# matchylabs/matchy

Hardware: AMD Instinct MI355X
Metric: log GB/s scanned (matchy match hot path, 100K IoCs) (higher is better)
Workload: dtype u8

## Files before the change

matchy_amd/csrc/device_common.h:

```cpp
#pragma once
#include <hip/hip_runtime.h>

#include "hashes.h"
#include "scan_types.h"

namespace mxy {

constexpr uint32_t C_B = 1, C_DIG = 2, C_DOT = 4, C_COLON = 8, C_AT = 16, C_LD = 32, C_NL = 64, C_TLD1 = 128;

constexpr uint64_t bnd_lo() {
    uint64_t m = 0;
    const int cs[] = {0x09, 0x0a, 0x0d, 0x20, 0x22, 0x27, 0x28, 0x29, 0x2c, 0x2f, 0x3a, 0x3b, 0x3c, 0x3d, 0x3e};
    for (int c : cs) m |= 1ull << c;
    return m;
}
constexpr uint64_t bnd_hi() {
    uint64_t m = 0;
    const int cs[] = {0x40, 0x5b, 0x5d, 0x7b, 0x7d};
    for (int c : cs) m |= 1ull << (c - 64);
    return m;
}
__device__ __forceinline__ bool d_is_boundary(uint32_t b) {
    if (b >= 128) return false;
    uint64_t m = b < 64 ? bnd_lo() : bnd_hi();
    return (m >> (b & 63)) & 1;
}
__device__ __forceinline__ bool d_is_digit(uint32_t b) { return b - '0' < 10u; }
__device__ __forceinline__ bool d_is_alpha(uint32_t b) { return (b | 0x20) - 'a' < 26u; }
__device__ __forceinline__ bool d_is_alnum(uint32_t b) { return d_is_digit(b) || d_is_alpha(b); }
__device__ __forceinline__ bool d_is_hex(uint32_t b) { return d_is_digit(b) || ((b | 0x20) - 'a' < 6u); }
__device__ __forceinline__ bool d_is_domain_char_fast(uint32_t b) { return d_is_alnum(b) || b == '-' || b == '.' || b >= 0x80; }
__device__ __forceinline__ bool d_is_domain_char(uint32_t b) { return d_is_alnum(b) || b == '-' || b == '.'; }
__device__ __forceinline__ bool d_is_email_local(uint32_t b) { return d_is_alnum(b) || b == '.' || b == '-' || b == '_' || b == '+'; }

__device__ __forceinline__ uint32_t class_of(uint32_t b) {
    uint32_t c = 0;
    if (d_is_boundary(b)) c |= C_B;
    if (d_is_digit(b)) c |= C_DIG;
    if (b == '.') c |= C_DOT;
    if (b == ':') c |= C_COLON;
    if (b == '@') c |= C_AT;
    if (d_is_alnum(b) || b >= 0x80) c |= C_LD;
    if (b == '\n') c |= C_NL;
    return c;
}

__device__ __forceinline__ uint32_t lane_id() { return __lane_id(); }
__device__ __forceinline__ uint64_t lanemask_lt() { return (1ull << lane_id()) - 1ull; }
__device__ __forceinline__ uint32_t mbcnt64_add(uint64_t m, uint32_t base) {
    return __builtin_amdgcn_mbcnt_hi((uint32_t)(m >> 32), __builtin_amdgcn_mbcnt_lo((uint32_t)m, base));
}
__device__ __forceinline__ uint32_t mbcnt64(uint64_t m) {
    return __builtin_amdgcn_mbcnt_hi((uint32_t)(m >> 32), __builtin_amdgcn_mbcnt_lo((uint32_t)m, 0u));
}

// ... 179 lines not shown
        const uint32_t n = (uint32_t)__popcll(m);
        if (left < n) {
            const uint32_t own = next == 0xFFFFFFFFu ? static_fn() : 0xFFFFFFFFu;
            pad_rest(out, cap);
            if (own != 0xFFFFFFFFu) {
                next = own;
                left = ANCHOR_CHUNK;
            } else {
                const uint32_t c = chunk_fn();
                uint32_t b = 0;
                uint32_t* const counter = counter_fn();
                if (lane_id() == 0) b = atomicAdd(counter, c);
                next = __builtin_amdgcn_readfirstlane(b);
                left = c;
            }
        }
        uint32_t slot = 0xFFFFFFFFu;
        if (emit) {
            slot = next + (uint32_t)__popcll(m & lanemask_lt());
            if (slot >= cap) slot = 0xFFFFFFFFu;
        }
        next += n;
        left -= n;
        return slot;
    }
};

struct LogView {
    const uint8_t* p;
    uint32_t len;
    __device__ __forceinline__ uint32_t at(uint32_t i) const { return p[i]; }
};

__device__ inline bool d_valid_utf8(const uint8_t* s, uint32_t n) {
    uint32_t i = 0;
    while (i < n) {
        uint32_t c = s[i];
        if (c < 0x80) { ++i; continue; }
        uint32_t l = (c >= 0xC2 && c <= 0xDF) ? 2 : (c >= 0xE0 && c <= 0xEF) ? 3 : (c >= 0xF0 && c <= 0xF4) ? 4 : 0;
        if (l == 0 || i + l > n) return false;
        uint32_t c1 = s[i + 1];
        uint32_t lo = 0x80, hi = 0xBF;
        if (c == 0xE0) lo = 0xA0;
        if (c == 0xED) hi = 0x9F;
        if (c == 0xF0) lo = 0x90;
        if (c == 0xF4) hi = 0x8F;
        if (c1 < lo || c1 > hi) return false;
        for (uint32_t k = 2; k < l; ++k) if ((s[i + k] & 0xC0) != 0x80) return false;
        i += l;
    }
    return true;
}

struct ByteMasks { uint64_t dc, dot, dash, high; };
struct ByteMasks32 { uint32_t dc, dot, dash, high; };
__device__ __forceinline__ ByteMasks32 domain_masks32(uint32_t x) {
    constexpr uint32_t H = 0x80808080u, L7 = 0x7F7F7F7Fu;
    const uint32_t t = x & L7, l = t | 0x20202020u;
    const uint32_t dig = (t + 0x50505050u) & ~(t + 0x46464646u);
    const uint32_t alp = (l + 0x1F1F1F1Fu) & ~(l + 0x05050505u);
    const uint32_t ndot = (t ^ 0x2E2E2E2Eu) + L7, ndash = (t ^ 0x2D2D2D2Du) + L7;
    ByteMasks32 m;
    m.high = x & H;
    m.dot = ~ndot & ~x & H;
    m.dash = ~ndash & ~x & H;
    m.dc = (((dig | alp) & ~x) | m.dot | m.dash | m.high) & H;
    return m;
}
__device__ __forceinline__ ByteMasks domain_masks(uint64_t x) {
    const ByteMasks32 lo = domain_masks32((uint32_t)x), hi = domain_masks32((uint32_t)(x >> 32));
    ByteMasks m;
    m.dc = (uint64_t)lo.dc | ((uint64_t)hi.dc << 32);
    m.dot = (uint64_t)lo.dot | ((uint64_t)hi.dot << 32);
    m.dash = (uint64_t)lo.dash | ((uint64_t)hi.dash << 32);
    m.high = (uint64_t)lo.high | ((uint64_t)hi.high << 32);
    return m;
}

__device__ __forceinline__ bool d_ipv4_from_window(uint4 q, uint32_t t4, uint32_t dot, uint32_t& start, uint32_t& end, uint32_t& addr) {
    const uint32_t b3 = q.x >> 24, b2 = (q.x >> 16) & 0xFF, b1 = (q.x >> 8) & 0xFF, b0 = q.x & 0xFF;
    if (!d_is_digit(b3)) return false;
    const bool g2 = d_is_digit(b2), g1 = g2 && d_is_digit(b1);
    const uint32_t n1 = 1u + g2 + g1;
    const uint32_t before = g1 ? b0 : g2 ? b1 : b2;
    if (!d_is_boundary(before)) return false;
    const uint32_t first = g1 ? b1 : g2 ? b2 : b3;
    uint32_t a = g1 ? (b1 - 48) * 100 + (b2 - 48) * 10 + (b3 - 48) : g2 ? (b2 - 48) * 10 + (b3 - 48) : (b3 - 48);
    if (a > 255 || (n1 > 1 && first == '0')) return false;
    uint32_t r0 = __builtin_amdgcn_alignbyte(q.z, q.y, 1), r1 = __builtin_amdgcn_alignbyte(q.w, q.z, 1), r2 = __builtin_amdgcn_alignbyte(t4, q.w, 1);
    uint32_t pos = dot + 1;
#pragma unroll
    for (int o = 0; o < 3; ++o) {
        const uint32_t c0 = r0 & 0xFF, c1 = (r0 >> 8) & 0xFF, c2 = (r0 >> 16) & 0xFF, c3 = r0 >> 24;
        if (!d_is_digit(c0)) return false;
        const bool h1 = d_is_digit(c1), h2 = h1 && d_is_digit(c2);
        const uint32_t n = 1u + h1 + h2;
        const uint32_t v = h2 ? (c0 - 48) * 100 + (c1 - 48) * 10 + (c2 - 48) : h1 ? (c0 - 48) * 10 + (c1 - 48) : (c0 - 48);
        if (v > 255 || (h1 && c0 == '0')) return false;
        const uint32_t sep = h2 ? c3 : h1 ? c2 : c1;
        a = (a << 8) | v;
        pos += n;
        if (o < 2) {
            if (sep != '.') return false;
            pos += 1;
            r0 = __builtin_amdgcn_alignbyte(r1, r0, n); r1 = __builtin_amdgcn_alignbyte(r2, r1, n); r2 = __builtin_amdgcn_alignbyte(0u, r2, n);
            r0 = __builtin_amdgcn_alignbyte(r1, r0, 1); r1 = __builtin_amdgcn_alignbyte(r2, r1, 1); r2 = r2 >> 8;
        } else if (!d_is_boundary(sep)) {
            return false;
        }
    }
    start = dot - n1; end = pos; addr = a;
    return true;
}
__device__ __forceinline__ bool val_ipv4_fast(const uint8_t* log, uint32_t dot, uint32_t& start, uint32_t& end, uint32_t& addr) {
    uint4 q;
    uint32_t t4;
    __builtin_memcpy(&q, log + dot - 4, 16);
    __builtin_memcpy(&t4, log + dot + 12, 4);
    return d_ipv4_from_window(q, t4, dot, start, end, addr);
}

__device__ inline bool val_ipv4(const LogView& lg, uint32_t dot, uint32_t& start, uint32_t& end, uint32_t& addr) {
    uint32_t s = dot;
    while (s > 0 && dot - s < 3 && d_is_digit(lg.at(s - 1))) --s;
    if (s == dot) return false;
    if (s > 0 && !d_is_boundary(lg.at(s - 1))) return false;
    uint32_t pos = s, a = 0;
    for (int idx = 0; idx < 4; ++idx) {
        uint32_t v = 0, digits = 0, first = 0;
        while (pos < lg.len && digits < 3) {
// ... 51 lines not shown
```

matchy_amd/csrc/hashes.h:

```cpp
#pragma once
#include <cstddef>
#include <cstdint>

#if defined(__HIPCC__)
#include <hip/hip_runtime.h>
#define MXY_HD __host__ __device__ inline __attribute__((always_inline))
#else
#define MXY_HD inline
#endif

namespace mxy {

MXY_HD uint64_t rotl64(uint64_t x, int r) { return (x << r) | (x >> (64 - r)); }

template <class Fetch>
MXY_HD uint64_t xxh64_fetch(Fetch f, size_t len, uint64_t seed) {
    const uint64_t P1 = 11400714785074694791ULL, P2 = 14029467366897019727ULL, P3 = 1609587929392839161ULL,
                   P4 = 9650029242287828579ULL, P5 = 2870177450012600261ULL;
    auto rd64 = [&](size_t o) {
        uint64_t v = 0;
        for (int k = 7; k >= 0; --k) v = (v << 8) | (uint64_t)f(o + k);
        return v;
    };
    auto rd32 = [&](size_t o) {
// ... 79 lines not shown
}

struct Xxh64Stream {
    static constexpr uint64_t P1 = 11400714785074694791ULL, P2 = 14029467366897019727ULL, P3 = 1609587929392839161ULL,
                              P4 = 9650029242287828579ULL, P5 = 2870177450012600261ULL;
    uint64_t v1, v2, v3, v4, lane[4] = {0, 0, 0, 0}, cur = 0, total = 0;
    uint32_t nlane = 0, ncur = 0;
    MXY_HD explicit Xxh64Stream(uint64_t seed) : v1(seed + P1 + P2), v2(seed + P2), v3(seed), v4(seed - P1) {}
    static MXY_HD uint64_t round(uint64_t acc, uint64_t in) { acc += in * P2; acc = rotl64(acc, 31); return acc * P1; }
    static MXY_HD uint64_t merge(uint64_t acc, uint64_t val) { val = round(0, val); acc ^= val; return acc * P1 + P4; }
    MXY_HD void push(uint32_t byte) {
        cur |= (uint64_t)(byte & 0xFF) << (8 * ncur);
        ++total;
        if (++ncur == 8) {
            lane[nlane] = cur; cur = 0; ncur = 0;
            if (++nlane == 4) {
                v1 = round(v1, lane[0]); v2 = round(v2, lane[1]); v3 = round(v3, lane[2]); v4 = round(v4, lane[3]);
                nlane = 0;
            }
        }
    }
    MXY_HD uint64_t finish(uint64_t seed) const {
        uint64_t h;
        if (total >= 32) {
            h = rotl64(v1, 1) + rotl64(v2, 7) + rotl64(v3, 12) + rotl64(v4, 18);
            h = merge(h, v1); h = merge(h, v2); h = merge(h, v3); h = merge(h, v4);
        } else {
            h = seed + P5;
        }
        h += total;
        for (uint32_t k = 0; k < nlane; ++k) { h ^= round(0, lane[k]); h = rotl64(h, 27) * P1 + P4; }
        uint64_t rest = cur;
        uint32_t n = ncur;
        if (n >= 4) { h ^= (rest & 0xFFFFFFFFull) * P1; h = rotl64(h, 23) * P2 + P3; rest >>= 32; n -= 4; }
        for (; n; --n) { h ^= (rest & 0xFF) * P5; h = rotl64(h, 11) * P1; rest >>= 8; }
        h ^= h >> 33; h *= P2; h ^= h >> 29; h *= P3; h ^= h >> 32;
        return h;
    }
};

MXY_HD uint32_t name_hash31(uint64_t l0, uint64_t l1, uint64_t l2, uint64_t l3, uint32_t n) {
    const uint64_t lane[4] = {l0, l1, l2, l3};
    uint32_t h = n * 0x9E3779B1u + 0x7F4A7C15u;
    for (int k = 0; k < 4; ++k) {
        const int rem = (int)n - 8 * k;
        const uint64_t m = rem >= 8 ? ~0ull : rem <= 0 ? 0ull : ((1ull << (8 * rem)) - 1ull);
        const uint64_t v = lane[k] & m;
        h = (h ^ (uint32_t)v) * 0x85EBCA6Bu; h ^= h >> 15;
        h = (h ^ (uint32_t)(v >> 32)) * 0xC2B2AE35u; h ^= h >> 13;
    }
    h *= 0x27D4EB2Fu; h ^= h >> 16;
    return h;
}

MXY_HD uint64_t fx_u32(uint32_t v) { return rotl64((uint64_t)v * 0xf1357aea2e62a9c5ULL, 26); }

constexpr uint32_t TLD_TAB_BITS = 11;
MXY_HD uint32_t tld_tab_slot(uint32_t lo, uint32_t hi24) { return ((lo ^ (hi24 * 0x9E3779B1u)) * 0x85EBCA6Bu) >> (32 - TLD_TAB_BITS); }

MXY_HD uint32_t tld_hash8(uint32_t lo, uint32_t hi) {
    uint32_t h = (lo * 0x9E3779B1u) ^ (hi * 0x85EBCA6Bu);
    h ^= h >> 16; h *= 0x7FEB352Du; h ^= h >> 15;
    return h;
}

MXY_HD uint64_t psl_hash_init() { return 0xcbf29ce484222325ULL; }
MXY_HD uint64_t psl_hash_step(uint64_t h, uint8_t b) { return (h ^ b) * 0x100000001b3ULL; }
MXY_HD uint64_t psl_hash_finish(uint64_t h) { h ^= h >> 29; h *= 0xbf58476d1ce4e5b9ULL; h ^= h >> 32; return h; }

}
```

matchy_amd/csrc/validate_kernels.hip:

```cpp
#include <hip/hip_runtime.h>

#include <cstdlib>

#include "hashes.h"
#include "scan_types.h"

#include "device_shared.h"

namespace mxy {


struct BackReader {
    const uint8_t* p;
    uint32_t pos;
    uint32_t cb;
    uint32_t k;
    uint64_t cur, nxt;
    __device__ __forceinline__ static uint64_t load8(const uint8_t* a) { uint64_t v; __builtin_memcpy(&v, a, 8); return v; }
    __device__ __forceinline__ void init(const uint8_t* base, uint32_t q) {
        p = base; pos = q; cb = 0; k = 0; cur = 0; nxt = 0;
        if (q >= 16) { cb = q - 8; k = 8; cur = load8(p + cb); nxt = load8(p + cb - 8); }
    }
    __device__ __forceinline__ uint32_t next() {
        --pos;
// ... 165 lines not shown
    }
    while (open && p < lg.len) {
        uint32_t c = lg.at(p);
        if (!d_is_domain_char_fast(c)) { stop_c = c; break; }
        if (c == '.') return false;
        if (p - j >= db.max_tld_len) return false;
        th = tld_hash_step(th, c);
        ++p;
    }
    const uint32_t e = p, ll = e - j;
    if (edge && stop_c == 0x100) *edge = true;
    if (ll > db.max_tld_len) return false;
    if (stop_c != 0x100 && !d_is_boundary(stop_c)) return false;
    bool alone = false;
    if (wide && ll <= 7) {
        const uint32_t lo = ll >= 4 ? w.x : (w.x & ((1u << (8 * ll)) - 1u));
        const uint32_t hi = ll > 4 ? (w.y & ((1u << (8 * (ll - 4))) - 1u)) : 0u;
        uint32_t slot = tld_tab_slot(lo, hi);
        for (;;) {
            const uint2 t = tldtab[slot];
            if ((t.y >> 24) == 0) return false;
            if (t.x == lo && (t.y & 0xFFFFFFu) == hi) { alone = (t.y >> 24) & 1; break; }
            slot = (slot + 1) & ((1u << TLD_TAB_BITS) - 1);
        }
    } else {
        const uint32_t bit = tld_hash_bit(th);
        if (!((bloom[bit >> 5] >> (bit & 31)) & 1)) return false;
    }
    uint32_t s;
    BackReader br;
    br.init(lg.p, e);
    WalkInit wi;
    wi.rh = psl_hash_init();
    WalkState ws{};
    const int r = alone ? domain_walk_back<false>(lg, db, min_labels, e, br, wi, s, long_out ? &ws : nullptr, nullptr, edge)
                        : domain_walk_back<true>(lg, db, min_labels, e, br, wi, s, long_out ? &ws : nullptr, nullptr, edge);
    if (r == WALK_LONG) { long_out->st = ws; long_out->e = e; long_out->alone = alone; return WALK_LONG; }
    if (r != WALK_YES) return WALK_NO;
    start = s; end = e;
    return WALK_YES;
}
__device__ bool val_domain_resume(const LogView& lg, const DevDb& db, uint32_t min_labels, const DomLong& dl, uint32_t& start, uint32_t& end, bool& need_utf8) {
    BackReader br;
    br.init(lg.p, dl.st.pos);
    WalkInit wi;
    wi.rh = psl_hash_init();
    wi.cur = dl.st.cur; wi.last_c = dl.st.last_c; wi.labels = dl.st.labels; wi.high = dl.st.high; wi.bad = dl.st.bad; wi.found = dl.st.found;
    uint32_t s;
    if (domain_walk_back<false>(lg, db, min_labels, dl.e, br, wi, s, nullptr, &need_utf8) != WALK_YES) return false;
    start = s; end = dl.e;
    return true;
}

__device__ __forceinline__ int val_domain_pre(const uint2* tldtab, uint32_t min_labels, uint32_t j, uint2 w, uint64_t b0, uint64_t b1,
                                              uint64_t b2, uint32_t& start, uint32_t& end) {
    constexpr uint64_t H = 0x8080808080808080ull;
    const uint64_t w64 = (uint64_t)w.x | ((uint64_t)w.y << 32);
    const ByteMasks mw = domain_masks(w64);
    const uint64_t ndc = ~mw.dc & H;
    const uint32_t ll = ndc ? (uint32_t)(__ffsll((long long)ndc) - 1) >> 3 : 8u;
    if (ll <= 7 && ll >= 1) {
        const uint64_t below = (1ull << (8 * ll)) - 1ull;
        if (mw.dot & below) return 0;
        const uint32_t stop_c = (uint32_t)(w64 >> (8 * ll)) & 0xFF;
        if (!d_is_boundary(stop_c)) return 0;
        const uint32_t lo = (uint32_t)(w64 & below), hi = (uint32_t)((w64 & below) >> 32);
        uint32_t slot = tld_tab_slot(lo, hi);
        bool alone = false;
        for (;;) {
            const uint2 t = tldtab[slot];
            if ((t.y >> 24) == 0) return 0;
            if (t.x == lo && (t.y & 0xFFFFFFu) == hi) { alone = (t.y >> 24) & 1; break; }
            slot = (slot + 1) & ((1u << TLD_TAB_BITS) - 1);
        }
        if (alone) {
            const ByteMasks m0 = domain_masks(b0), m1 = domain_masks(b1), m2 = domain_masks(b2);
            const uint64_t n0m = ~m0.dc & H, n1m = ~m1.dc & H, n2m = ~m2.dc & H;
            const uint32_t c0 = n0m ? (uint32_t)__clzll((long long)n0m) >> 3 : 8u;
            const uint32_t c1 = n1m ? (uint32_t)__clzll((long long)n1m) >> 3 : 8u, c2 = n2m ? (uint32_t)__clzll((long long)n2m) >> 3 : 8u;
            const uint32_t consumed = c0 < 8 ? c0 : (c1 < 8 ? 8 + c1 : 16 + c2);
            if (consumed < 24 || j == 24) {
                auto top = [](uint32_t k) -> uint64_t { return k == 0 ? 0ull : (~0ull << (64 - 8 * k)); };
                const uint64_t r0 = top(min(consumed, 8u)), r1 = top(consumed > 8 ? min(consumed - 8, 8u) : 0u),
                               r2 = top(consumed > 16 ? consumed - 16 : 0u);
                const uint64_t d0 = m0.dot >> 8, d1 = (m1.dot >> 8) | (m0.dot << 56), d2 = (m2.dot >> 8) | (m1.dot << 56);
                const uint64_t s0 = m0.dash >> 8, s1 = (m1.dash >> 8) | (m0.dash << 56), s2 = (m2.dash >> 8) | (m1.dash << 56);
                const uint64_t bad = ((m0.dot & (d0 | s0)) | (m0.dash & d0)) & r0;
                const uint64_t bad1 = ((m1.dot & (d1 | s1)) | (m1.dash & d1)) & r1, bad2 = ((m2.dot & (d2 | s2)) | (m2.dash & d2)) & r2;
                const uint32_t ndots = (uint32_t)(__popcll(m0.dot & r0) + __popcll(m1.dot & r1) + __popcll(m2.dot & r2));
                const uint32_t li = 24 - consumed;
                const uint64_t lw = li < 8 ? b2 : li < 16 ? b1 : b0;
                const uint32_t left_c = (uint32_t)(lw >> (8 * (li & 7))) & 0xFF;
                const uint32_t fi = 23 - consumed;
                const uint64_t fw = fi < 8 ? b2 : fi < 16 ? b1 : b0;
                const uint32_t first_c = consumed < 24 ? (uint32_t)(fw >> (8 * (fi & 7))) & 0xFF : 0x100u;
                const uint32_t lastc = (uint32_t)(w64 >> (8 * (ll - 1))) & 0xFF;
                const bool any_bad = (bad | bad1 | bad2) != 0 || lastc == '-' || consumed == 0 || left_c == '.' || left_c == '-';
                if (any_bad || ndots == 0 || 1 + ndots < min_labels) return 0;
                if (first_c != 0x100 && !d_is_boundary(first_c)) return 0;
                const uint32_t s_pos = j - consumed;
                const bool high = ((m0.high & r0) | (m1.high & r1) | (m2.high & r2) | (mw.high & below)) != 0;
                if (high) return 2;
                start = s_pos; end = j + ll;
                return 1;
            }
        }
    }
    return 2;
}

template <int NB>
__device__ __forceinline__ int val_domain_ctx(const uint2* tldtab, uint32_t min_labels, uint32_t j, uint2 w, const uint64_t (&b)[NB],
                                              uint32_t& start, uint32_t& end) {
    static_assert(NB >= 1 && NB <= 7, "a label must not reach 64 bytes inside the context");
    constexpr uint64_t H = 0x8080808080808080ull;
    const uint64_t w64 = (uint64_t)w.x | ((uint64_t)w.y << 32);
    const ByteMasks mw = domain_masks(w64);
    const uint64_t ndc = ~mw.dc & H;
    const uint32_t ll = ndc ? (uint32_t)(__ffsll((long long)ndc) - 1) >> 3 : 8u;
    if (ll > 7 || ll < 1) return 2;
    const uint64_t below = (1ull << (8 * ll)) - 1ull;
    if (mw.dot & below) return 0;
    const uint32_t stop_c = (uint32_t)(w64 >> (8 * ll)) & 0xFF;
    if (!d_is_boundary(stop_c)) return 0;
    const uint32_t lo = (uint32_t)(w64 & below), hi = (uint32_t)((w64 & below) >> 32);
    uint32_t slot = tld_tab_slot(lo, hi);
    bool alone = false;
    for (;;) {
        const uint2 t = tldtab[slot];
        if ((t.y >> 24) == 0) return 0;
        if (t.x == lo && (t.y & 0xFFFFFFu) == hi) { alone = (t.y >> 24) & 1; break; }
        slot = (slot + 1) & ((1u << TLD_TAB_BITS) - 1);
    }
    if (!alone) return 2;
    ByteMasks m[NB];
    uint32_t consumed = 0;
    bool open = true;
#pragma unroll
    for (int k = 0; k < NB; ++k) {
        m[k] = domain_masks(b[k]);
        const uint64_t nm = ~m[k].dc & H;
        const uint32_t ck = nm ? (uint32_t)__clzll((long long)nm) >> 3 : 8u;
        if (open) { consumed += ck; open = ck == 8; }
    }
    if (consumed == 8 * NB && j != 8 * NB) return 2;
    uint64_t bad = 0, high = mw.high & below;
    uint32_t ndots = 0;
#pragma unroll
    for (int k = 0; k < NB; ++k) {
        const uint32_t in_k = consumed > 8u * k ? min(consumed - 8u * k, 8u) : 0u;
        const uint64_t r = in_k == 0 ? 0ull : (~0ull << (64 - 8 * in_k));
        const uint64_t d = (m[k].dot >> 8) | (k ? (m[k ? k - 1 : 0].dot << 56) : 0ull);
        const uint64_t sd = (m[k].dash >> 8) | (k ? (m[k ? k - 1 : 0].dash << 56) : 0ull);
        bad |= ((m[k].dot & (d | sd)) | (m[k].dash & d)) & r;
        ndots += (uint32_t)__popcll(m[k].dot & r);
        high |= m[k].high & r;
    }
    const uint32_t li = 8 * NB - consumed, fi = li - 1;
    uint32_t left_c = 0, first_c = 0x100u;
#pragma unroll
    for (int k = 0; k < NB; ++k) {
        const uint32_t wi = (uint32_t)(NB - 1 - k);
// ... 421 lines not shown
    d_keccak256_1blk(dec, dl - 4, h);
    const uint32_t chk = (uint32_t)dec[dl - 4] | ((uint32_t)dec[dl - 3] << 8) | ((uint32_t)dec[dl - 2] << 16) | ((uint32_t)dec[dl - 1] << 24);
    return (uint32_t)h[0] == chk;
}
__device__ int d_bech32_val(uint32_t c) {
    const char* CS = "qpzry9x8gf2tvdw0s3jn54khce6mua7l";
    for (int i = 0; i < 32; ++i) if ((uint32_t)CS[i] == c) return i;
    return -1;
}
__device__ bool val_btc_bech32(const uint8_t* s, uint32_t n) {
    if (n < 3 + 6) return false;
    auto step = [](uint32_t chk, uint32_t v) {
        const uint32_t GEN[5] = {0x3b6a57b2, 0x26508e6d, 0x1ea119fa, 0x3d4233dd, 0x2a1462b3};
        uint32_t top = chk >> 25;
        chk = ((chk & 0x1ffffff) << 5) ^ v;
        for (int i = 0; i < 5; ++i) if ((top >> i) & 1) chk ^= GEN[i];
        return chk;
    };
    uint32_t chk = 1;
    chk = step(chk, 'b' >> 5); chk = step(chk, 'c' >> 5); chk = step(chk, 0); chk = step(chk, 'b' & 31); chk = step(chk, 'c' & 31);
    for (uint32_t k = 3; k < n; ++k) {
        int v = d_bech32_val(s[k]);
        if (v < 0) return false;
        chk = step(chk, (uint32_t)v);
    }
    return chk == 1 || chk == 0x2bc830a3u;
}
__device__ bool val_eth(const uint8_t* a, uint8_t* lower) {
    bool all_lower = true, all_upper = true;
    for (int i = 0; i < 40; ++i) {
        uint32_t c = a[2 + i];
        if (!d_is_hex(c)) return false;
        if (d_is_alpha(c)) { if (c >= 'a') all_upper = false; else all_lower = false; }
        lower[i] = (uint8_t)d_lower(c);
    }
    if (all_lower || all_upper) return true;
    uint64_t h[4];
    d_keccak256_1blk(lower, 40, h);
    for (int i = 0; i < 40; ++i) {
        uint32_t c = a[2 + i];
        if (d_is_alpha(c)) {
            const uint32_t byte = (uint32_t)(h[i >> 4] >> (8 * ((i >> 1) & 7))) & 0xFF;
            const uint32_t nib = (i & 1) ? (byte & 0x0f) : (byte >> 4);
            if ((c < 'a') != (nib >= 8)) return false;
        }
    }
    return true;
}

template <int MODE>
__global__ __launch_bounds__(256) void k_validate_dom(TokParams p, DevDb db) {
    constexpr bool AC = MODE == 1, SFX = MODE == 2;
    __shared__ uint2 tldtab[1u << TLD_TAB_BITS];
    __shared__ __attribute__((aligned(16))) uint32_t strbuf[256][8];
    __shared__ uint8_t dcls[AC ? 256 : 4];
    __shared__ uint32_t drows[AC ? DFA_LDS_ENTRIES_VAL : 1];
    for (uint32_t i = threadIdx.x; i < (1u << TLD_TAB_BITS); i += blockDim.x) tldtab[i] = db.tld_tab[i];
    DfaView dv{dcls, drows, 0};
    if constexpr (AC) dv = dfa_stage<DFA_LDS_ENTRIES_VAL>(db, dcls, drows);
    __syncthreads();
    ChunkWriter<Candidate, CAND_CHUNK> cw_dense;
    __shared__ Candidate wb_cand[4][64];
    BufferedWriter<Candidate> cw(wb_cand[threadIdx.x >> 6]);
    __shared__ RareAnchor wb_slow[4][64];
    BufferedWriter<RareAnchor> sw(wb_slow[threadIdx.x >> 6]);
    const Candidate SC{0, 0xFFFFFFFFu, 0, 0};
    const uint32_t stride = gridDim.x * blockDim.x;
    const uint32_t nd = min(p.counters->n_dom, p.dom_cap);
    struct Rec { uint32_t j; uint32_t c[8]; };
    auto load_rec = [&](uint32_t i, Rec& r) {
        r.j = 0xFFFFFFFFu;
#pragma unroll
        for (int k = 0; k < 8; ++k) r.c[k] = 0;
        if (i < nd) {
            r.j = p.dom_list[dom_plane_index(i, 0)];
#pragma unroll
            for (int k = 0; k < 8; ++k) r.c[k] = p.dom_list[dom_plane_index(i, 1 + k)];
        }
    };
    Rec cur, nxt;
    load_rec(blockIdx.x * blockDim.x + threadIdx.x, cur);
    {
        uint32_t g = cur.j;
#pragma unroll
        for (int k = 0; k < 8; ++k) g ^= cur.c[k];
        asm volatile("" ::"v"(g));
    }
    uint32_t pend_start = 0, pend_lt = 0, pend_word = 0xFFFFFFFFu, pend_bit = 0, n_valid = 0;
    uint32_t pend_sw[SFX ? 4 : 1] = {0}, pend_sb[SFX ? 4 : 1] = {0};
    bool pend = false, pend_over = false;
    uint32_t* sb = strbuf[threadIdx.x];
    auto queue_glob = [&](uint32_t b, uint32_t n) {
        if (!p.glob_work_d) return;
        const uint32_t lane = lane_id();
        const bool g = lane < n && b + lane < p.cand_cap && cw.buf[lane].pad == CAND_GLOB;
        const uint64_t m = __ballot(g);
        if (!m) return;
        uint32_t wb = 0;
        if (lane == 0) wb = atomicAdd(&p.counters->n_glob_work_d, (uint32_t)__popcll(m));
        wb = __builtin_amdgcn_readfirstlane(wb);
        const uint32_t slot = wb + mbcnt64(m);
        if (g && slot < p.glob_work_d_cap) p.glob_work_d[slot] = b + lane;
    };
    auto emit_pending = [&]() {
        if (!p.filter_lit) { cw_dense.append(pend, Candidate{pend_start, pend_lt, 0u, 0u}, p.cands, p.cand_cap, p.n_cand, SC); return; }
        bool lit = (pend_word >> pend_bit) & 1;
        uint32_t flag = 0;
        if constexpr (SFX) {
            bool g = pend_over;
#pragma unroll
            for (int q = 0; q < 4; ++q) g = g || ((pend_sw[q] >> pend_sb[q]) & 1);
            flag = g ? CAND_GLOB : CAND_NO_GLOB;
            lit = lit || g;
        }
        if constexpr (AC) flag = pend_over ? CAND_GLOB : CAND_NO_GLOB;
        if constexpr (AC || SFX) cw.append_then(pend && lit, Candidate{pend_start, pend_lt, 0u, flag}, p.cands, p.cand_cap, p.n_cand, queue_glob);
        else cw.append(pend && lit, Candidate{pend_start, pend_lt, 0u, flag}, p.cands, p.cand_cap, p.n_cand);
    };
    for (uint32_t base = blockIdx.x * blockDim.x; base < nd; base += stride) {
        const uint32_t i = base + threadIdx.x;
        emit_pending();
        pend = false;
        load_rec(i + stride, nxt);
        bool slow = false;
        if (cur.j != 0xFFFFFFFFu) {
            uint32_t s = 0, e = 0;
            int r = 2;
            if (!(cur.j & 0x80000000u)) {
                const uint64_t b2 = (uint64_t)cur.c[0] | ((uint64_t)cur.c[1] << 32), b1 = (uint64_t)cur.c[2] | ((uint64_t)cur.c[3] << 32),
                               b0 = (uint64_t)cur.c[4] | ((uint64_t)cur.c[5] << 32);
                r = val_domain_pre(tldtab, p.min_labels, cur.j, make_uint2(cur.c[6], cur.c[7]), b0, b1, b2, s, e);
            }
            slow = r == 2;
            if (r == 1) {
                pend_start = s; pend_lt = (e - s) | ((uint32_t)IT_DOMAIN << 24); pend = true;
                pend_word = 0xFFFFFFFFu; pend_bit = 0;
                n_valid += 1;
                if (p.filter_lit) {
                    *reinterpret_cast<uint4*>(sb) = make_uint4(cur.c[0], cur.c[1], cur.c[2], cur.c[3]);
                    *reinterpret_cast<uint4*>(sb + 4) = make_uint4(cur.c[4], cur.c[5], cur.c[6], cur.c[7]);
                    const uint32_t o = 24 - (cur.j - s), n = e - s;
                    const uint32_t i0 = o >> 2, sh = o & 3;
                    uint32_t wd[9];
#pragma unroll
                    for (int k = 0; k < 9; ++k) wd[k] = (i0 + k) < 8 ? sb[(i0 + k) & 7] : 0u;
                    uint64_t ln[4];
#pragma unroll
                    for (int k = 0; k < 4; ++k)
                        ln[k] = (uint64_t)__builtin_amdgcn_alignbyte(wd[2 * k + 1], wd[2 * k], sh) |
                                ((uint64_t)__builtin_amdgcn_alignbyte(wd[2 * k + 2], wd[2 * k + 1], sh) << 32);
                    if (db.ci) {
#pragma unroll
                        for (int k = 0; k < 4; ++k) ln[k] = ascii_lower8(ln[k]);
                    }
                    const uint32_t b = name_hash31(ln[0], ln[1], ln[2], ln[3], n) & db.lit_bm_mask;
                    pend_word = db.lit_bm ? db.lit_bm[b >> 5] : 0u;
                    pend_bit = b & 31;
                    if constexpr (SFX) {
                        const uint64_t fb = 0x0101010101010101ull * db.sfx_first;
                        uint32_t M = 0;
#pragma unroll
                        for (int k = 0; k < 4; ++k) {
                            const uint64_t x = ln[k] ^ fb;
                            const uint64_t z = ~(((x & 0x7F7F7F7F7F7F7F7Full) + 0x7F7F7F7F7F7F7F7Full) | x) & 0x8080808080808080ull;
                            const uint32_t lo = (uint32_t)z >> 7, hi = (uint32_t)(z >> 32) >> 7;
                            M |= ((((lo * 0x01020408u) >> 24) & 0xFu) | ((((hi * 0x01020408u) >> 24) & 0xFu) << 4)) << (8 * k);
                        }
                        M &= n >= 32 ? 0xFFFFFFFFu : ((1u << n) - 1u);
                        pend_over = false;
                        uint32_t dm = db.sfx_dots;
#pragma unroll
                        for (int q = 0; q < 4; ++q) {
                            pend_sw[q] = 0; pend_sb[q] = 0;
                            if (dm) {
                                const uint32_t d = (uint32_t)__builtin_ctz(dm) + 1;
                                dm &= dm - 1;
                                uint32_t m = M;
                                for (uint32_t j = 1; j < d; ++j) m &= ~(m ? (0x80000000u >> __builtin_clz(m)) : 0u);
                                if (m) {
                                    const uint32_t kk = 31u - (uint32_t)__builtin_clz(m), sl = n - kk;
                                    if (sl >= 3) {
                                        const uint32_t o2 = o + kk, j0 = o2 >> 2, s2 = o2 & 3;
                                        uint32_t w2[9];
#pragma unroll
                                        for (int k = 0; k < 9; ++k) w2[k] = (j0 + k) < 8 ? sb[(j0 + k) & 7] : 0u;
                                        uint64_t l2[4];
#pragma unroll
                                        for (int k = 0; k < 4; ++k)
                                            l2[k] = (uint64_t)__builtin_amdgcn_alignbyte(w2[2 * k + 1], w2[2 * k], s2) |
                                                    ((uint64_t)__builtin_amdgcn_alignbyte(w2[2 * k + 2], w2[2 * k + 1], s2) << 32);
                                        if (db.ci) {
#pragma unroll
                                            for (int k = 0; k < 4; ++k) l2[k] = ascii_lower8(l2[k]);
                                        }
                                        const uint32_t b2 = name_hash31(l2[0], l2[1], l2[2], l2[3], sl) & db.sfx_mask;
                                        pend_sw[q] = db.sfx_bm[b2 >> 5];
                                        pend_sb[q] = b2 & 31;
                                    }
                                }
                            }
                        }
                    }
                    if constexpr (AC) {
                        uint32_t st = 0, any = 0;
#pragma unroll
                        for (int k = 0; k < 31; ++k) {
                            const uint32_t c = dcls[(uint32_t)(ln[k >> 3] >> (8 * (k & 7))) & 0xFF];
                            if ((uint32_t)k < n) {
                                const uint32_t t = st < dv.lds_states ? drows[st * db.dfa_k + c] : db.dfa[(size_t)st * db.dfa_k + c];
                                st = t & 0x7FFFFFFFu;
                                any |= t;
                            }
                        }
                        pend_over = (any >> 31) != 0;
                        if (pend_over) { pend_word = 0xFFFFFFFFu; pend_bit = 0; }
                    }
                }
            }
        }
        sw.append(slow, RareAnchor{cur.j & 0x7FFFFFFFu, (uint32_t)RARE_DOM}, p.rare_dom, p.rare_dom_cap, &p.counters->n_rare_dom);
        cur = nxt;
    }
    emit_pending();
    if constexpr (AC || SFX) cw.flush_then(p.cands, p.cand_cap, p.n_cand, queue_glob);
    else cw.flush(p.cands, p.cand_cap, p.n_cand);
    cw_dense.pad_rest(p.cands, p.cand_cap, SC);
    sw.flush(p.rare_dom, p.rare_dom_cap, &p.counters->n_rare_dom);
#pragma unroll
    for (int off = 32; off > 0; off >>= 1) n_valid += __shfl_down(n_valid, off);
    if (lane_id() == 0 && n_valid) atomicAdd(&p.counters->cand_true, n_valid);
}

__device__ __forceinline__ bool lit_bm_may_hit(const DevDb& db, const LogView& lg, uint32_t s, uint32_t n, bool ascii) {
    uint64_t l[4] = {0, 0, 0, 0};
    if (s + 32 <= lg.len) {
#pragma unroll
        for (int k = 0; k < 4; ++k) __builtin_memcpy(&l[k], lg.p + s + 8 * k, 8);
    } else {
        for (uint32_t k = 0; k < 32 && s + k < lg.len; ++k) l[k >> 3] |= (uint64_t)lg.p[s + k] << (8 * (k & 7));
    }
    if (db.ci) {
        if (!ascii) {
            if (n > 32) return true;
            uint64_t high = 0;
#pragma unroll
            for (int k = 0; k < 4; ++k) {
                const int rem = (int)n - 8 * k;
                const uint64_t m = rem >= 8 ? ~0ull : (rem <= 0 ? 0ull : ((1ull << (8 * rem)) - 1ull));
// ... 373 lines not shown
```

Measured before the change: 2236.

## Rewrite domain pre-validation with bit-plane masks and register-only label alignment

```diff
diff --git a/matchy_amd/csrc/device_common.h b/matchy_amd/csrc/device_common.h
--- a/matchy_amd/csrc/device_common.h
+++ b/matchy_amd/csrc/device_common.h
@@ -1,6 +1,7 @@
 #pragma once
 #include <hip/hip_runtime.h>
 
+#include "domain_pre.h"
 #include "hashes.h"
 #include "scan_types.h"
 
@@ -286,30 +287,6 @@
     return true;
 }
 
-struct ByteMasks { uint64_t dc, dot, dash, high; };
-struct ByteMasks32 { uint32_t dc, dot, dash, high; };
-__device__ __forceinline__ ByteMasks32 domain_masks32(uint32_t x) {
-    constexpr uint32_t H = 0x80808080u, L7 = 0x7F7F7F7Fu;
-    const uint32_t t = x & L7, l = t | 0x20202020u;
-    const uint32_t dig = (t + 0x50505050u) & ~(t + 0x46464646u);
-    const uint32_t alp = (l + 0x1F1F1F1Fu) & ~(l + 0x05050505u);
-    const uint32_t ndot = (t ^ 0x2E2E2E2Eu) + L7, ndash = (t ^ 0x2D2D2D2Du) + L7;
-    ByteMasks32 m;
-    m.high = x & H;
-    m.dot = ~ndot & ~x & H;
-    m.dash = ~ndash & ~x & H;
-    m.dc = (((dig | alp) & ~x) | m.dot | m.dash | m.high) & H;
-    return m;
-}
-__device__ __forceinline__ ByteMasks domain_masks(uint64_t x) {
-    const ByteMasks32 lo = domain_masks32((uint32_t)x), hi = domain_masks32((uint32_t)(x >> 32));
-    ByteMasks m;
-    m.dc = (uint64_t)lo.dc | ((uint64_t)hi.dc << 32);
-    m.dot = (uint64_t)lo.dot | ((uint64_t)hi.dot << 32);
-    m.dash = (uint64_t)lo.dash | ((uint64_t)hi.dash << 32);
-    m.high = (uint64_t)lo.high | ((uint64_t)hi.high << 32);
-    return m;
-}
 
 __device__ __forceinline__ bool d_ipv4_from_window(uint4 q, uint32_t t4, uint32_t dot, uint32_t& start, uint32_t& end, uint32_t& addr) {
     const uint32_t b3 = q.x >> 24, b2 = (q.x >> 16) & 0xFF, b1 = (q.x >> 8) & 0xFF, b0 = q.x & 0xFF;
diff --git a/matchy_amd/csrc/domain_pre.h b/matchy_amd/csrc/domain_pre.h
--- /dev/null
+++ b/matchy_amd/csrc/domain_pre.h
@@ -0,0 +1,139 @@
+#pragma once
+#include <cstdint>
+
+#include "anchor_planes.h"
+#include "hashes.h"
+
+namespace mxy {
+
+struct ByteMasks { uint64_t dc, dot, dash, high; };
+struct ByteMasks32 { uint32_t dc, dot, dash, high; };
+MXY_HD ByteMasks32 domain_masks32(uint32_t x) {
+    constexpr uint32_t H = 0x80808080u, L7 = 0x7F7F7F7Fu;
+    const uint32_t t = x & L7, l = t | 0x20202020u;
+    const uint32_t dig = (t + 0x50505050u) & ~(t + 0x46464646u);
+    const uint32_t alp = (l + 0x1F1F1F1Fu) & ~(l + 0x05050505u);
+    const uint32_t ndot = (t ^ 0x2E2E2E2Eu) + L7, ndash = (t ^ 0x2D2D2D2Du) + L7;
+    ByteMasks32 m;
+    m.high = x & H;
+    m.dot = ~ndot & ~x & H;
+    m.dash = ~ndash & ~x & H;
+    m.dc = (((dig | alp) & ~x) | m.dot | m.dash | m.high) & H;
+    return m;
+}
+MXY_HD ByteMasks domain_masks(uint64_t x) {
+    const ByteMasks32 lo = domain_masks32((uint32_t)x), hi = domain_masks32((uint32_t)(x >> 32));
+    ByteMasks m;
+    m.dc = (uint64_t)lo.dc | ((uint64_t)hi.dc << 32);
+    m.dot = (uint64_t)lo.dot | ((uint64_t)hi.dot << 32);
+    m.dash = (uint64_t)lo.dash | ((uint64_t)hi.dash << 32);
+    m.high = (uint64_t)lo.high | ((uint64_t)hi.high << 32);
+    return m;
+}
+
+MXY_HD uint32_t byte_perm(uint32_t hi, uint32_t lo, uint32_t sel) {
+#if defined(__HIP_DEVICE_COMPILE__)
+    return __builtin_amdgcn_perm(hi, lo, sel);
+#else
+    const uint64_t v = ((uint64_t)hi << 32) | lo;
+    uint32_t r = 0;
+    for (int i = 0; i < 4; ++i) r |= (uint32_t)((v >> (8 * ((sel >> (8 * i)) & 7))) & 0xFF) << (8 * i);
+    return r;
+#endif
+}
+MXY_HD uint32_t byte_align(uint32_t hi, uint32_t lo, uint32_t sh) {
+#if defined(__HIP_DEVICE_COMPILE__)
+    return __builtin_amdgcn_alignbyte(hi, lo, sh);
+#else
+    return (uint32_t)((((uint64_t)hi << 32) | lo) >> (8 * (sh & 3)));
+#endif
+}
+
+struct CtxMasks {
+    uint32_t dc;
+    uint32_t dot;
+    uint32_t dash;
+    uint32_t high;
+    uint32_t bnd;
+};
+MXY_HD CtxMasks domain_ctx_masks(const uint32_t (&c)[8]) {
+    uint32_t r[8];
+#pragma unroll
+    for (int h = 0; h < 2; ++h) {
+        const uint32_t x0 = byte_perm(c[2 + h], c[h], 0x05010400u), x1 = byte_perm(c[2 + h], c[h], 0x07030602u);
+        const uint32_t y0 = byte_perm(c[6 + h], c[4 + h], 0x05010400u), y1 = byte_perm(c[6 + h], c[4 + h], 0x07030602u);
+        r[4 * h + 0] = byte_perm(y0, x0, 0x05040100u);
+        r[4 * h + 1] = byte_perm(y0, x0, 0x07060302u);
+        r[4 * h + 2] = byte_perm(y1, x1, 0x05040100u);
+        r[4 * h + 3] = byte_perm(y1, x1, 0x07060302u);
+    }
+    bit_transpose8(r);
+    const ClassPlanes cp = classify_planes(r, false);
+    CtxMasks m;
+    m.high = r[7];
+    m.dot = cp.T;
+    m.dash = andn(r[7] | r[6] | r[4] | r[1], r[5] & r[3] & r[2] & r[0]);
+    m.dc = cp.LD | cp.T | m.dash;
+    m.bnd = cp.B;
+    return m;
+}
+
+MXY_HD uint32_t ctx_label_len(const CtxMasks& m) { return (uint32_t)__builtin_ctz(~(m.dc >> 24)); }
+MXY_HD uint32_t ctx_label_lo(uint32_t w0, uint32_t ll) { return ll >= 4 ? w0 : (w0 & ((1u << (8 * ll)) - 1u)); }
+MXY_HD uint32_t ctx_label_hi(uint32_t w1, uint32_t ll) { return ll > 4 ? (w1 & ((1u << (8 * (ll - 4))) - 1u)) : 0u; }
+
+template <class TldEntry>
+MXY_HD int val_domain_pre(const TldEntry* tldtab, uint32_t min_labels, uint32_t j, const uint32_t (&c)[8], const CtxMasks& m,
+                          uint32_t& start, uint32_t& end) {
+    constexpr uint32_t FRONT = 0x00FFFFFFu;
+    const uint32_t ll = ctx_label_len(m);
+    if (ll > 7 || ll < 1) return 2;
+    const uint32_t lab = ((1u << ll) - 1u) << 24;
+    if (m.dot & lab) return 0;
+    if (!((m.bnd >> (24 + ll)) & 1u)) return 0;
+    const uint32_t lo = ctx_label_lo(c[6], ll), hi = ctx_label_hi(c[7], ll);
+    uint32_t slot = tld_tab_slot(lo, hi);
+    bool alone = false;
+    for (;;) {
+        const TldEntry t = tldtab[slot];
+        if ((t.y >> 24) == 0) return 0;
+        if (t.x == lo && (t.y & 0xFFFFFFu) == hi) { alone = (t.y >> 24) & 1; break; }
+        slot = (slot + 1) & ((1u << TLD_TAB_BITS) - 1);
+    }
+    if (!alone) return 2;
+    const uint32_t ndc = ~m.dc & FRONT;
+    const uint32_t consumed = ndc ? (uint32_t)__builtin_clz(ndc) - 8u : 24u;
+    if (consumed == 24 && j != 24) return 2;
+    const uint32_t li = 24 - consumed;
+    const uint32_t reg = FRONT & ~((1u << li) - 1u);
+    const uint32_t dash = m.dash & FRONT;
+    const uint32_t dr = m.dot >> 1, sr = dash >> 1;
+    const uint32_t bad = ((m.dot & (dr | sr)) | (dash & dr)) & reg;
+    const uint32_t ndots = (uint32_t)__builtin_popcount(m.dot & reg);
+    const uint32_t left_bad = ((m.dot | dash) >> (li & 31)) & 1u;
+    const uint32_t last_dash = (m.dash >> (23 + ll)) & 1u;
+    if (bad != 0 || last_dash || consumed == 0 || left_bad || ndots == 0 || 1 + ndots < min_labels) return 0;
+    if (consumed < 24 && !((m.bnd >> (23 - consumed)) & 1u)) return 0;
+    if (m.high & (reg | lab)) return 2;
+    start = j - consumed; end = j + ll;
+    return 1;
+}
+
+MXY_HD void ctx_align(const uint32_t (&c)[8], uint32_t o, uint64_t (&ln)[4]) {
+    const uint32_t sh = o & 3;
+    const uint32_t m0 = 0u - ((o >> 2) & 1u), m1 = 0u - ((o >> 3) & 1u), m2 = 0u - ((o >> 4) & 1u);
+    const uint32_t a0 = byte_align(c[1], c[0], sh), a1 = byte_align(c[2], c[1], sh), a2 = byte_align(c[3], c[2], sh), a3 = byte_align(c[4], c[3], sh),
+                   a4 = byte_align(c[5], c[4], sh), a5 = byte_align(c[6], c[5], sh), a6 = byte_align(c[7], c[6], sh), a7 = byte_align(0u, c[7], sh);
+    const uint32_t s0 = bsel(m0, a1, a0), s1 = bsel(m0, a2, a1), s2 = bsel(m0, a3, a2), s3 = bsel(m0, a4, a3), s4 = bsel(m0, a5, a4),
+                   s5 = bsel(m0, a6, a5), s6 = bsel(m0, a7, a6), s7 = andn(m0, a7);
+    const uint32_t t0 = bsel(m1, s2, s0), t1 = bsel(m1, s3, s1), t2 = bsel(m1, s4, s2), t3 = bsel(m1, s5, s3), t4 = bsel(m1, s6, s4),
+                   t5 = bsel(m1, s7, s5), t6 = andn(m1, s6), t7 = andn(m1, s7);
+    const uint32_t u0 = bsel(m2, t4, t0), u1 = bsel(m2, t5, t1), u2 = bsel(m2, t6, t2), u3 = bsel(m2, t7, t3), u4 = andn(m2, t4),
+                   u5 = andn(m2, t5), u6 = andn(m2, t6), u7 = andn(m2, t7);
+    ln[0] = (uint64_t)u0 | ((uint64_t)u1 << 32);
+    ln[1] = (uint64_t)u2 | ((uint64_t)u3 << 32);
+    ln[2] = (uint64_t)u4 | ((uint64_t)u5 << 32);
+    ln[3] = (uint64_t)u6 | ((uint64_t)u7 << 32);
+}
+
+}
diff --git a/matchy_amd/csrc/hashes.h b/matchy_amd/csrc/hashes.h
--- a/matchy_amd/csrc/hashes.h
+++ b/matchy_amd/csrc/hashes.h
@@ -155,6 +155,16 @@
     h *= 0x27D4EB2Fu; h ^= h >> 16;
     return h;
 }
+MXY_HD uint32_t name_hash31_zp(uint64_t l0, uint64_t l1, uint64_t l2, uint64_t l3, uint32_t n) {
+    const uint64_t lane[4] = {l0, l1, l2, l3};
+    uint32_t h = n * 0x9E3779B1u + 0x7F4A7C15u;
+    for (int k = 0; k < 4; ++k) {
+        h = (h ^ (uint32_t)lane[k]) * 0x85EBCA6Bu; h ^= h >> 15;
+        h = (h ^ (uint32_t)(lane[k] >> 32)) * 0xC2B2AE35u; h ^= h >> 13;
+    }
+    h *= 0x27D4EB2Fu; h ^= h >> 16;
+    return h;
+}
 
 MXY_HD uint64_t fx_u32(uint32_t v) { return rotl64((uint64_t)v * 0xf1357aea2e62a9c5ULL, 26); }
 
diff --git a/matchy_amd/csrc/validate_kernels.hip b/matchy_amd/csrc/validate_kernels.hip
--- a/matchy_amd/csrc/validate_kernels.hip
+++ b/matchy_amd/csrc/validate_kernels.hip
@@ -241,62 +241,6 @@
     return true;
 }
 
-__device__ __forceinline__ int val_domain_pre(const uint2* tldtab, uint32_t min_labels, uint32_t j, uint2 w, uint64_t b0, uint64_t b1,
-                                              uint64_t b2, uint32_t& start, uint32_t& end) {
-    constexpr uint64_t H = 0x8080808080808080ull;
-    const uint64_t w64 = (uint64_t)w.x | ((uint64_t)w.y << 32);
-    const ByteMasks mw = domain_masks(w64);
-    const uint64_t ndc = ~mw.dc & H;
-    const uint32_t ll = ndc ? (uint32_t)(__ffsll((long long)ndc) - 1) >> 3 : 8u;
-    if (ll <= 7 && ll >= 1) {
-        const uint64_t below = (1ull << (8 * ll)) - 1ull;
-        if (mw.dot & below) return 0;
-        const uint32_t stop_c = (uint32_t)(w64 >> (8 * ll)) & 0xFF;
-        if (!d_is_boundary(stop_c)) return 0;
-        const uint32_t lo = (uint32_t)(w64 & below), hi = (uint32_t)((w64 & below) >> 32);
-        uint32_t slot = tld_tab_slot(lo, hi);
-        bool alone = false;
-        for (;;) {
-            const uint2 t = tldtab[slot];
-            if ((t.y >> 24) == 0) return 0;
-            if (t.x == lo && (t.y & 0xFFFFFFu) == hi) { alone = (t.y >> 24) & 1; break; }
-            slot = (slot + 1) & ((1u << TLD_TAB_BITS) - 1);
-        }
-        if (alone) {
-            const ByteMasks m0 = domain_masks(b0), m1 = domain_masks(b1), m2 = domain_masks(b2);
-            const uint64_t n0m = ~m0.dc & H, n1m = ~m1.dc & H, n2m = ~m2.dc & H;
-            const uint32_t c0 = n0m ? (uint32_t)__clzll((long long)n0m) >> 3 : 8u;
-            const uint32_t c1 = n1m ? (uint32_t)__clzll((long long)n1m) >> 3 : 8u, c2 = n2m ? (uint32_t)__clzll((long long)n2m) >> 3 : 8u;
-            const uint32_t consumed = c0 < 8 ? c0 : (c1 < 8 ? 8 + c1 : 16 + c2);
-            if (consumed < 24 || j == 24) {
-                auto top = [](uint32_t k) -> uint64_t { return k == 0 ? 0ull : (~0ull << (64 - 8 * k)); };
-                const uint64_t r0 = top(min(consumed, 8u)), r1 = top(consumed > 8 ? min(consumed - 8, 8u) : 0u),
-                               r2 = top(consumed > 16 ? consumed - 16 : 0u);
-                const uint64_t d0 = m0.dot >> 8, d1 = (m1.dot >> 8) | (m0.dot << 56), d2 = (m2.dot >> 8) | (m1.dot << 56);
-                const uint64_t s0 = m0.dash >> 8, s1 = (m1.dash >> 8) | (m0.dash << 56), s2 = (m2.dash >> 8) | (m1.dash << 56);
-                const uint64_t bad = ((m0.dot & (d0 | s0)) | (m0.dash & d0)) & r0;
-                const uint64_t bad1 = ((m1.dot & (d1 | s1)) | (m1.dash & d1)) & r1, bad2 = ((m2.dot & (d2 | s2)) | (m2.dash & d2)) & r2;
-                const uint32_t ndots = (uint32_t)(__popcll(m0.dot & r0) + __popcll(m1.dot & r1) + __popcll(m2.dot & r2));
-                const uint32_t li = 24 - consumed;
-                const uint64_t lw = li < 8 ? b2 : li < 16 ? b1 : b0;
-                const uint32_t left_c = (uint32_t)(lw >> (8 * (li & 7))) & 0xFF;
-                const uint32_t fi = 23 - consumed;
-                const uint64_t fw = fi < 8 ? b2 : fi < 16 ? b1 : b0;
-                const uint32_t first_c = consumed < 24 ? (uint32_t)(fw >> (8 * (fi & 7))) & 0xFF : 0x100u;
-                const uint32_t lastc = (uint32_t)(w64 >> (8 * (ll - 1))) & 0xFF;
-                const bool any_bad = (bad | bad1 | bad2) != 0 || lastc == '-' || consumed == 0 || left_c == '.' || left_c == '-';
-                if (any_bad || ndots == 0 || 1 + ndots < min_labels) return 0;
-                if (first_c != 0x100 && !d_is_boundary(first_c)) return 0;
-                const uint32_t s_pos = j - consumed;
-                const bool high = ((m0.high & r0) | (m1.high & r1) | (m2.high & r2) | (mw.high & below)) != 0;
-                if (high) return 2;
-                start = s_pos; end = j + ll;
-                return 1;
-            }
-        }
-    }
-    return 2;
-}
 
 template <int NB>
 __device__ __forceinline__ int val_domain_ctx(const uint2* tldtab, uint32_t min_labels, uint32_t j, uint2 w, const uint64_t (&b)[NB],
@@ -824,7 +768,6 @@
 __global__ __launch_bounds__(256) void k_validate_dom(TokParams p, DevDb db) {
     constexpr bool AC = MODE == 1, SFX = MODE == 2;
     __shared__ uint2 tldtab[1u << TLD_TAB_BITS];
-    __shared__ __attribute__((aligned(16))) uint32_t strbuf[256][8];
     __shared__ uint8_t dcls[AC ? 256 : 4];
     __shared__ uint32_t drows[AC ? DFA_LDS_ENTRIES_VAL : 1];
     for (uint32_t i = threadIdx.x; i < (1u << TLD_TAB_BITS); i += blockDim.x) tldtab[i] = db.tld_tab[i];
@@ -837,6 +780,11 @@
     __shared__ RareAnchor wb_slow[4][64];
     BufferedWriter<RareAnchor> sw(wb_slow[threadIdx.x >> 6]);
     const Candidate SC{0, 0xFFFFFFFFu, 0, 0};
+#ifdef MXY_VDOM_DEBUG
+    const uint32_t dbg = p.debug;
+#else
+    constexpr uint32_t dbg = 0;
+#endif
     const uint32_t stride = gridDim.x * blockDim.x;
     const uint32_t nd = min(p.counters->n_dom, p.dom_cap);
     struct Rec { uint32_t j; uint32_t c[8]; };
@@ -861,7 +809,6 @@
     uint32_t pend_start = 0, pend_lt = 0, pend_word = 0xFFFFFFFFu, pend_bit = 0, n_valid = 0;
     uint32_t pend_sw[SFX ? 4 : 1] = {0}, pend_sb[SFX ? 4 : 1] = {0};
     bool pend = false, pend_over = false;
-    uint32_t* sb = strbuf[threadIdx.x];
     auto queue_glob = [&](uint32_t b, uint32_t n) {
         if (!p.glob_work_d) return;
         const uint32_t lane = lane_id();
@@ -891,42 +838,36 @@
     };
     for (uint32_t base = blockIdx.x * blockDim.x; base < nd; base += stride) {
         const uint32_t i = base + threadIdx.x;
-        emit_pending();
+        if (!(dbg & 4)) emit_pending();
         pend = false;
         load_rec(i + stride, nxt);
         bool slow = false;
         if (cur.j != 0xFFFFFFFFu) {
             uint32_t s = 0, e = 0;
             int r = 2;
-            if (!(cur.j & 0x80000000u)) {
-                const uint64_t b2 = (uint64_t)cur.c[0] | ((uint64_t)cur.c[1] << 32), b1 = (uint64_t)cur.c[2] | ((uint64_t)cur.c[3] << 32),
-                               b0 = (uint64_t)cur.c[4] | ((uint64_t)cur.c[5] << 32);
-                r = val_domain_pre(tldtab, p.min_labels, cur.j, make_uint2(cur.c[6], cur.c[7]), b0, b1, b2, s, e);
-            }
+            if (dbg & 1) { r = 1; s = cur.j - 9; e = cur.j + 1; }
+            else if (!(cur.j & 0x80000000u)) r = val_domain_pre(tldtab, p.min_labels, cur.j, cur.c, domain_ctx_masks(cur.c), s, e);
             slow = r == 2;
             if (r == 1) {
                 pend_start = s; pend_lt = (e - s) | ((uint32_t)IT_DOMAIN << 24); pend = true;
                 pend_word = 0xFFFFFFFFu; pend_bit = 0;
                 n_valid += 1;
                 if (p.filter_lit) {
-                    *reinterpret_cast<uint4*>(sb) = make_uint4(cur.c[0], cur.c[1], cur.c[2], cur.c[3]);
-                    *reinterpret_cast<uint4*>(sb + 4) = make_uint4(cur.c[4], cur.c[5], cur.c[6], cur.c[7]);
+                    const uint32_t ll = e - cur.j;
+                    const uint32_t nc[8] = {cur.c[0], cur.c[1], cur.c[2], cur.c[3], cur.c[4], cur.c[5], ctx_label_lo(cur.c[6], ll), ctx_label_hi(cur.c[7], ll)};
                     const uint32_t o = 24 - (cur.j - s), n = e - s;
-                    const uint32_t i0 = o >> 2, sh = o & 3;
-                    uint32_t wd[9];
-#pragma unroll
-                    for (int k = 0; k < 9; ++k) wd[k] = (i0 + k) < 8 ? sb[(i0 + k) & 7] : 0u;
-                    uint64_t ln[4];
-#pragma unroll
-                    for (int k = 0; k < 4; ++k)
-                        ln[k] = (uint64_t)__builtin_amdgcn_alignbyte(wd[2 * k + 1], wd[2 * k], sh) |
-                                ((uint64_t)__builtin_amdgcn_alignbyte(wd[2 * k + 2], wd[2 * k + 1], sh) << 32);
-                    if (db.ci) {
-#pragma unroll
-                        for (int k = 0; k < 4; ++k) ln[k] = ascii_lower8(ln[k]);
+                    uint64_t ln[4] = {0, 0, 0, 0};
+                    uint32_t b = cur.j;
+                    if (!(dbg & 2)) {
+                        ctx_align(nc, o, ln);
+                        if (db.ci) {
+#pragma unroll
+                            for (int k = 0; k < 4; ++k) ln[k] = ascii_lower8(ln[k]);
+                        }
+                        b = name_hash31_zp(ln[0], ln[1], ln[2], ln[3], n);
                     }
-                    const uint32_t b = name_hash31(ln[0], ln[1], ln[2], ln[3], n) & db.lit_bm_mask;
-                    pend_word = db.lit_bm ? db.lit_bm[b >> 5] : 0u;
+                    b &= db.lit_bm_mask;
+                    pend_word = db.lit_bm && !(dbg & 4) ? db.lit_bm[b >> 5] : 0u;
                     pend_bit = b & 31;
                     if constexpr (SFX) {
                         const uint64_t fb = 0x0101010101010101ull * db.sfx_first;
@@ -952,20 +893,13 @@
                                 if (m) {
                                     const uint32_t kk = 31u - (uint32_t)__builtin_clz(m), sl = n - kk;
                                     if (sl >= 3) {
-                                        const uint32_t o2 = o + kk, j0 = o2 >> 2, s2 = o2 & 3;
-                                        uint32_t w2[9];
-#pragma unroll
-                                        for (int k = 0; k < 9; ++k) w2[k] = (j0 + k) < 8 ? sb[(j0 + k) & 7] : 0u;
                                         uint64_t l2[4];
-#pragma unroll
-                                        for (int k = 0; k < 4; ++k)
-                                            l2[k] = (uint64_t)__builtin_amdgcn_alignbyte(w2[2 * k + 1], w2[2 * k], s2) |
-                                                    ((uint64_t)__builtin_amdgcn_alignbyte(w2[2 * k + 2], w2[2 * k + 1], s2) << 32);
+                                        ctx_align(nc, o + kk, l2);
                                         if (db.ci) {
 #pragma unroll
                                             for (int k = 0; k < 4; ++k) l2[k] = ascii_lower8(l2[k]);
                                         }
-                                        const uint32_t b2 = name_hash31(l2[0], l2[1], l2[2], l2[3], sl) & db.sfx_mask;
+                                        const uint32_t b2 = name_hash31_zp(l2[0], l2[1], l2[2], l2[3], sl) & db.sfx_mask;
                                         pend_sw[q] = db.sfx_bm[b2 >> 5];
                                         pend_sb[q] = b2 & 31;
                                     }
```

New measurement: 2266 (median of 6 runs). +1.3%, better.
